# hyf015/egocentric-gaze-prediction

Hardware: AMD Instinct MI355X
Metric: SP+AT train frames/sec/node (224x224, bs32/GPU) (higher is better)
Workload: dtype f32 (every convolution -- forward, data gradient, weight gradient -- as f16 split-half MFMA, abs-max scaled operands, THREE products per MAC: 22 significant bits on both operands of every product; fp32 accumulate; everything else exact f32)

## Files before the change

### egocentric-gaze-prediction_amd/_lib.py

```python
from __future__ import annotations

import ctypes
import os
from ctypes import c_char_p, c_double, c_float, c_int, c_long, c_size_t, c_void_p

_HERE = os.path.dirname(os.path.abspath(__file__))
LIB_PATH = os.environ.get("EGAZE_HIP_LIB") or os.path.join(_HERE, "csrc", "libegaze_hip.so")

P = c_void_p
S = c_void_p

SIGNATURES = {
    "egz_version": (c_char_p, []),
    "egz_last_error": (c_char_p, []),
    "egz_mfma_probe": (c_int, [P, P, c_int, c_int, S]),
    "egz_u8_center_of_mass": (c_int, [P, c_int, c_int, c_int, P, P, P, S]),
    "egz_bilinear_up": (c_int, [P, P, c_int, c_int, c_int, c_int, c_int, c_long, S]),
    "egz_pack_w3x3_elems": (c_size_t, [c_int, c_int, c_int]),
    "egz_pack_w3x3_ups_fwd": (c_int, [P, P, c_int, c_int, S]),
    "egz_pack_w3x3_ups_dgrad": (c_int, [P, P, c_int, c_int, S]),
    "egz_conv3x3_ups_dgrad": (c_int, [P, P, P, c_int, c_int, c_int, c_int, c_int, c_int, S]),
    "egz_pack_w3x3_fwd": (c_int, [P, P, c_int, c_int, S]),
    "egz_pack_w3x3_dgrad": (c_int, [P, P, c_int, c_int, S]),
    "egz_conv3x3_stat_rows": (c_int, [c_int, c_int, c_int, c_int, c_int]),
# ... 91 lines not shown
    "egz_gaze_gt_maps": (c_int, [P, c_int, c_int, c_int, P, c_int, P, P, P, c_int, P, P, P, c_int, c_int, c_int, c_int,
                                 P, P, P, S]),
    "egz_resize_linear_u8": (c_int, [P, c_int, c_int, c_int, c_int, c_int, c_int, c_int, P, P, P, P, P, S]),
    "egz_heatmap_overlay": (c_int, [P, c_int, c_int, c_int, P, P, c_int, c_int, c_int, P, P, P, P, P, P, S]),
    "egz_cell_argmax_u8": (c_int, [P, c_int, c_int, c_int, c_int, P, S]),
    "egz_jpeg_decode_ws_bytes": (c_size_t, [c_int, c_int, c_int, c_int]),
    "egz_jpeg_decode": (c_int, [P, c_long, P, P, P, c_int, c_int, c_int, P, c_long, P, P, c_size_t, c_int, c_int, S]),
    "egz_jpeg_encode_ws_bytes": (c_size_t, [c_int, c_int, c_int, c_int]),
    "egz_jpeg_encode": (c_int, [P, c_int, c_int, c_int, c_int, c_int, c_int, P, c_size_t, P, c_int, S]),
    "egz_jpeg_encode_write": (c_int, [P, c_size_t, c_int, c_int, c_int, c_int, P, c_long, P, P, P, P, S]),
    "egz_tvl1_default_k": (c_int, []),
    "egz_bgr_to_gray_u8": (c_int, [P, c_int, c_int, c_int, c_int, P, S]),
    "egz_flow_gauss": (c_int, [P, c_int, c_int, c_int, c_int, P, c_int, P, P, S]),
    "egz_flow_resample": (c_int, [P, c_int, c_int, c_int, P, c_int, c_int, c_float, S]),
    "egz_flow_grad": (c_int, [P, c_int, c_int, c_int, P, P, S]),
    "egz_tvl1_warp": (c_int, [P, P, P, P, P, c_int, c_int, c_int, S]),
    "egz_tvl1_iterate": (c_int, [P, P, P, c_int, c_int, c_int, c_int, c_int, c_double, c_double, c_double, S]),
    "egz_flow_to_u8": (c_int, [P, c_long, c_double, P, S]),
    "egz_tvl1_flow_ws_bytes": (c_size_t, [c_int, c_int, c_int, c_int, c_double]),
    "egz_tvl1_flow": (c_int, [P, c_int, c_int, c_int, P, c_int, P, c_int, c_double, c_double, c_double, c_int, c_double,
                              c_int, c_int, c_int, P, c_size_t, P, P, S]),
    "egz_adam_step": (c_int, [P, P, P, P, c_long, c_double, c_double, c_double, c_double, c_int, c_double, P, S]),
    "egz_adam_step_dev": (c_int, [P, P, P, P, c_long, c_double, c_double, c_double, c_double, P, c_double, P, S]),
}


class EgazeHipError(RuntimeError):
    """Raised when a C-ABI entry point returns a non-zero code (mirrors the reference's convention of
    plain Python exceptions: utils.generalException / RuntimeError, SURVEY.md 8b)."""


def _load():
    if not os.path.exists(LIB_PATH):
        raise ImportError(
            f"{LIB_PATH} is missing: the HIP extension is mandatory (no CPU fallback). "
            "Build it with `python __graft_entry__.py` or `csrc/build.sh`.")
    import torch
    lib = ctypes.CDLL(LIB_PATH)
    for name, (res, args) in SIGNATURES.items():
        try:
            fn = getattr(lib, name)
        except AttributeError as e:
            raise ImportError(f"{LIB_PATH} does not export {name}; rebuild the extension") from e
        fn.restype = res
        fn.argtypes = args
    return lib
# ... 14 lines not shown
```

### egocentric-gaze-prediction_amd/csrc/adam.hip

```cpp
#include "egz_common.h"

namespace {
__global__ __launch_bounds__(256) void adam_kernel(float* __restrict__ p, const float* __restrict__ g, float* __restrict__ m,
                                                   float* __restrict__ v, long n, float omb1, float beta2, float omb2, float eps,
                                                   float step_size, float bc2_sqrt, float grad_scale,
                                                   unsigned int* __restrict__ nonfinite) {
#pragma clang fp contract(off)
    const long n4 = n >> 2;
    bool bad = false;
    for (long i = blockIdx.x * (long)blockDim.x + threadIdx.x; i < n4; i += (long)gridDim.x * blockDim.x) {
        f32x4 pv = reinterpret_cast<f32x4*>(p)[i];
        const f32x4 gv = reinterpret_cast<const f32x4*>(g)[i];
        f32x4 mv = reinterpret_cast<f32x4*>(m)[i];
        f32x4 vv = reinterpret_cast<f32x4*>(v)[i];
#pragma unroll
        for (int e = 0; e < 4; ++e) {
            const float ge = gv[e] * grad_scale;
            if (!(fabsf(ge) <= 3.402823466e38f)) { bad = true; continue; }
            mv[e] = mv[e] + omb1 * (ge - mv[e]);
            vv[e] = vv[e] * beta2 + omb2 * ge * ge;
            const float denom = sqrtf(vv[e]) / bc2_sqrt + eps;
            pv[e] = pv[e] - step_size * (mv[e] / denom);
        }
        reinterpret_cast<f32x4*>(p)[i] = pv;
        reinterpret_cast<f32x4*>(m)[i] = mv;
        reinterpret_cast<f32x4*>(v)[i] = vv;
    }
    const long t = n4 * 4 + blockIdx.x * (long)blockDim.x + threadIdx.x;
    if (t < n) {
        const float ge = g[t] * grad_scale;
        if (!(fabsf(ge) <= 3.402823466e38f)) bad = true;
        else {
            const float mm = m[t] + omb1 * (ge - m[t]);
            const float vq = v[t] * beta2 + omb2 * ge * ge;
            m[t] = mm;
            v[t] = vq;
            p[t] = p[t] - step_size * (mm / (sqrtf(vq) / bc2_sqrt + eps));
        }
    }
    if (bad && nonfinite) atomicOr(nonfinite, 1u);
}
__global__ __launch_bounds__(256) void adam_dev_kernel(float* __restrict__ p, const float* __restrict__ g, float* __restrict__ m,
                                                       float* __restrict__ v, long n, double lr, double beta1, double beta2,
                                                       float eps, int* __restrict__ step, float grad_scale,
                                                       unsigned int* __restrict__ nonfinite) {
#pragma clang fp contract(off)
    bool bad = false;
    const double t = (double)(*static_cast<volatile int*>(step) + 1);
    const float omb1 = (float)(1.0 - beta1), b2 = (float)beta2, omb2 = (float)(1.0 - beta2);
    const float step_size = (float)(lr / (1.0 - pow(beta1, t)));
    const float bc2_sqrt = (float)sqrt(1.0 - pow(beta2, t));
    const long n4 = n >> 2;
    for (long i = blockIdx.x * (long)blockDim.x + threadIdx.x; i < n4; i += (long)gridDim.x * blockDim.x) {
        f32x4 pv = reinterpret_cast<f32x4*>(p)[i];
        const f32x4 gv = reinterpret_cast<const f32x4*>(g)[i];
        f32x4 mv = reinterpret_cast<f32x4*>(m)[i];
        f32x4 vv = reinterpret_cast<f32x4*>(v)[i];
#pragma unroll
        for (int e = 0; e < 4; ++e) {
            const float ge = gv[e] * grad_scale;
            if (!(fabsf(ge) <= 3.402823466e38f)) { bad = true; continue; }
            mv[e] = mv[e] + omb1 * (ge - mv[e]);
            vv[e] = vv[e] * b2 + omb2 * ge * ge;
            const float denom = sqrtf(vv[e]) / bc2_sqrt + eps;
            pv[e] = pv[e] - step_size * (mv[e] / denom);
        }
        reinterpret_cast<f32x4*>(p)[i] = pv;
        reinterpret_cast<f32x4*>(m)[i] = mv;
        reinterpret_cast<f32x4*>(v)[i] = vv;
    }
    const long tl = n4 * 4 + blockIdx.x * (long)blockDim.x + threadIdx.x;
    if (tl < n) {
        const float ge = g[tl] * grad_scale;
        if (!(fabsf(ge) <= 3.402823466e38f)) bad = true;
        else {
            const float mm = m[tl] + omb1 * (ge - m[tl]);
            const float vq = v[tl] * b2 + omb2 * ge * ge;
            m[tl] = mm;
            v[tl] = vq;
            p[tl] = p[tl] - step_size * (mm / (sqrtf(vq) / bc2_sqrt + eps));
        }
    }
    if (bad && nonfinite) atomicOr(nonfinite, 1u);
}
__global__ void adam_bump_kernel(int* step) { *step += 1; }
}

EGZ_API int egz_adam_step_dev(float* p, const float* g, float* m, float* v, long n, double lr, double beta1, double beta2,
                              double eps, int* step, double grad_scale, unsigned int* nonfinite, hipStream_t st) {
    EGZ_CHECK_ARG(p && g && m && v && step && n > 0, "egz_adam_step_dev: bad arguments");
    EGZ_CHECK_ARG(((uintptr_t)p % 16 == 0) && ((uintptr_t)g % 16 == 0) && ((uintptr_t)m % 16 == 0) && ((uintptr_t)v % 16 == 0),
                  "egz_adam_step_dev: buffers must be 16-byte aligned");
    long g4 = (n / 4 + 255) / 256;
    if (g4 < 1) g4 = 1;
    const int grid = (int)(g4 > 8192 ? 8192 : g4);
    hipLaunchKernelGGL(adam_dev_kernel, dim3(grid), dim3(256), 0, st, p, g, m, v, n, lr, beta1, beta2, (float)eps, step,
                       (float)grad_scale, nonfinite);
    EGZ_CHECK_LAUNCH("egz_adam_step_dev");
    hipLaunchKernelGGL(adam_bump_kernel, dim3(1), dim3(1), 0, st, step);
    EGZ_CHECK_LAUNCH("egz_adam_step_dev(bump)");
    return 0;
}

EGZ_API int egz_adam_step(float* p, const float* g, float* m, float* v, long n, double lr, double beta1, double beta2,
                          double eps, int step, double grad_scale, unsigned int* nonfinite, hipStream_t st) {
    EGZ_CHECK_ARG(p && g && m && v && n > 0 && step >= 1, "egz_adam_step: bad arguments");
    EGZ_CHECK_ARG(((uintptr_t)p % 16 == 0) && ((uintptr_t)g % 16 == 0) && ((uintptr_t)m % 16 == 0) && ((uintptr_t)v % 16 == 0),
                  "egz_adam_step: buffers must be 16-byte aligned");
    const double bc1 = 1.0 - pow(beta1, (double)step);
    const double bc2 = 1.0 - pow(beta2, (double)step);
    const float step_size = (float)(lr / bc1);
    const float bc2_sqrt = (float)sqrt(bc2);
    long g4 = (n / 4 + 255) / 256;
    if (g4 < 1) g4 = 1;
    const int grid = (int)(g4 > 8192 ? 8192 : g4);
    hipLaunchKernelGGL(adam_kernel, dim3(grid), dim3(256), 0, st, p, g, m, v, n,
                       (float)(1.0 - beta1), (float)beta2, (float)(1.0 - beta2), (float)eps, step_size, bc2_sqrt, (float)grad_scale, nonfinite);
    EGZ_CHECK_LAUNCH("egz_adam_step");
    return 0;
}
```

### egocentric-gaze-prediction_amd/csrc/conv3x3_igemm_x3s.hip

```cpp
#include "egz_common.h"
#include "x3_split.h"
#include <type_traits>



namespace {
using namespace x3;

enum { EPI_BIAS = 0, EPI_BIAS_RELU = 1, EPI_BIAS_STATS = 2, EPI_MASK_SUMS = 3, EPI_PARTIAL = 4, EPI_BNSUMS = 5 };
constexpr int XLD = 32;
constexpr int XBK = 32;
constexpr int HPITCH = 20;

template <int WM> struct Geo {
    static constexpr int WMM = WM;
    static constexpr int NWN = 4 / WM;
    static constexpr int NTHR = 64 * WMM * NWN;
    static constexpr int MR = (WM == 4) ? 2 : 4;
    static constexpr int RPW = 32 * MR;
    static constexpr int BM = RPW * WMM, BN = 32 * NWN;
    static constexpr int HSLOTS = (WM == 1) ? 256 : 384, HZERO = HSLOTS - 1;
    static constexpr int NABUF = (WM == 1) ? 2 : 1;
    static constexpr int PROWS = BM / 16;
    static constexpr int SPP = NTHR / 8;
// ... 550 lines not shown
            const long srow = (long)tile_m * G::WMM + wm;
            if (hl == 0 && nok && srow * 128 < M) {
                stat[(srow * 2 + 0) * K + col] = s1;
                stat[(srow * 2 + 1) * K + col] = s2;
            }
        } else {
            if (hl == 0) {
                sred[(wave * 2 + 0) * 32 + l31] = s1;
                sred[(wave * 2 + 1) * 32 + l31] = s2;
            }
            lds_barrier();
            const long srow = (long)tile_m * (BM / 128) + (wm >> 1);
            if ((wm & 1) == 0 && hl == 0 && nok && srow * 128 < M) {
                stat[(srow * 2 + 0) * K + col] = s1 + sred[((wave + NWN) * 2 + 0) * 32 + l31];
                stat[(srow * 2 + 1) * K + col] = s2 + sred[((wave + NWN) * 2 + 1) * 32 + l31];
            }
        }
    }
#ifdef EGZ_TILE_LOOP
    }
#endif
}

__device__ __forceinline__ float weff9s(const float* __restrict__ w9, int py, int a, int px, int b) {
    const int rlo = (py == 0) ? (a == 0 ? 0 : 1) : (a == 0 ? 0 : 2), rhi = (py == 0) ? (a == 0 ? 0 : 2) : (a == 0 ? 1 : 2);
    const int slo = (px == 0) ? (b == 0 ? 0 : 1) : (b == 0 ? 0 : 2), shi = (px == 0) ? (b == 0 ? 0 : 2) : (b == 0 ? 1 : 2);
    float s = 0.f;
    for (int r = rlo; r <= rhi; ++r)
        for (int q = slo; q <= shi; ++q) s += w9[r * 3 + q];
    return s;
}

__device__ __forceinline__ float frag_value9(const float* w9, int kind, int si) {
    if (kind == 4) return w9[si];
    if (kind == 5) return w9[8 - si];
    if (kind == 7) return weff9s(w9, (si >> 2) >> 1, (si & 3) >> 1, (si >> 2) & 1, si & 1);
    const int img = si >> 2, tap = si & 3;
    const int oy = 2 * (tap >> 1) - (img >> 1), ox = 2 * (tap & 1) - (img & 1);
    return weff9s(w9, (oy == -1 || oy == 1) ? 1 : 0, (oy <= 0) ? 1 : 0, (ox == -1 || ox == 1) ? 1 : 0, (ox <= 0) ? 1 : 0);
}

template <typename T, int KIND>
__device__ __forceinline__ void frag_pack_pair(const float* __restrict__ w, unsigned short* __restrict__ wq, int C, int K,
                                               int Np, int Rp, float scale, long j) {
    constexpr int NS = (KIND >= 6) ? 16 : 9;
    const int nt32 = Np >> 5, ncb = Rp / XBK;
    const int e = (int)(j & 7), lane = (int)((j >> 3) & 63), ks = (int)((j >> 9) & 1);
    const long r2 = j >> 10;
    const int ntile = (int)(r2 % nt32), cblk = (int)(r2 / nt32);
    const int col = ntile * 32 + (lane & 31), k = cblk * XBK + ks * 16 + (lane >> 5) * 8 + e;
    float w9[9];
    const bool fwd = (KIND == 4 || KIND == 7);
    const bool ok = fwd ? (col < K && k < C) : (col < C && k < K);
    const float* src = w + (fwd ? ((long)col * C + k) : ((long)k * C + col)) * 9;
#pragma unroll
    for (int t = 0; t < 9; ++t) w9[t] = ok ? src[t] : 0.f;
#pragma unroll
    for (int si = 0; si < NS; ++si) {
        const long s = (KIND == 7) ? (long)(si >> 2) * (ncb * 4) + cblk * 4 + (si & 3) : (long)cblk * NS + si;
        const long r = s * nt32 + ntile;
        unsigned short h, l;
        Half<T>::split(frag_value9(w9, KIND, si) * scale, h, l);
        const long base = ((r * 2 + ks) * 2) * 512 + lane * 8 + e;
        wq[base] = h;
        wq[base + 512] = l;
    }
}
template <typename T>
__device__ __forceinline__ void frag_pack_pair_k(const float* __restrict__ w, unsigned short* __restrict__ wq, int C, int K,
                                                 int kind, int Np, int Rp, float scale, long j) {
    if (kind == 4) frag_pack_pair<T, 4>(w, wq, C, K, Np, Rp, scale, j);
    else if (kind == 5) frag_pack_pair<T, 5>(w, wq, C, K, Np, Rp, scale, j);
    else if (kind == 6) frag_pack_pair<T, 6>(w, wq, C, K, Np, Rp, scale, j);
    else frag_pack_pair<T, 7>(w, wq, C, K, Np, Rp, scale, j);
}

template <typename T>
__global__ __launch_bounds__(256) void pack_split_frag_kernel(const float* __restrict__ w, unsigned short* __restrict__ wq,
                                                             int C, int K, int kind, int Np, int Rp, float scale) {
    const long n = (long)Np * Rp;
    for (long j = blockIdx.x * (long)blockDim.x + threadIdx.x; j < n; j += (long)gridDim.x * blockDim.x)
        frag_pack_pair_k<T>(w, wq, C, K, kind, Np, Rp, scale, j);
}


constexpr int PT_LD = 289;
template <typename T>
__device__ __forceinline__ void pack_frag_tile(const float* __restrict__ w, unsigned short* __restrict__ wq, int C, int K,
                                               int kind, float scale, int tile, float* __restrict__ sw) {
    const int Cp = (C + 31) & ~31, Kp = (K + 31) & ~31;
    const int ncbc = Cp >> 5;
    const int kb = tile / ncbc, cb = tile - kb * ncbc;
    const int tid = threadIdx.x;
    if (C % 32 == 0 && (reinterpret_cast<unsigned long long>(w) & 15) == 0) {
        for (int idx = tid; idx < 32 * 72; idx += 256) {
            const int i = idx / 72, q = idx - i * 72;
            const int k = kb * 32 + i;
            f32x4 v = f32x4{0.f, 0.f, 0.f, 0.f};
            if (k < K) v = *reinterpret_cast<const f32x4*>(w + ((long)k * C + cb * 32) * 9 + q * 4);
            float* d = sw + i * PT_LD + q * 4;
            d[0] = v[0]; d[1] = v[1]; d[2] = v[2]; d[3] = v[3];
        }
    } else {
        for (int idx = tid; idx < 32 * 288; idx += 256) {
            const int i = idx / 288, q = idx - i * 288;
            const int k = kb * 32 + i, c = cb * 32 + q / 9;
            sw[i * PT_LD + q] = (k < K && c < C) ? w[(long)k * C * 9 + cb * 288 + q] : 0.f;
        }
    }
    __syncthreads();
    const bool fwd = (kind == 4 || kind == 7);
    const int NS = (kind >= 6) ? 16 : 9;
    const int nt32 = (fwd ? Kp : Cp) >> 5, ncb = (fwd ? Cp : Kp) >> 5;
    const int ntile = fwd ? kb : cb, cblk = fwd ? cb : kb;
    for (int it = tid; it < NS * 128; it += 256) {
        const int lane = it & 63, ks = (it >> 6) & 1, si = it >> 7;
        const int col = lane & 31, kk0 = ks * 16 + (lane >> 5) * 8;
        const float* p = fwd ? sw + col * PT_LD + kk0 * 9 : sw + kk0 * PT_LD + col * 9;
        const int estep = fwd ? 9 : PT_LD;
        unsigned short h[8], l[8];
#pragma unroll
        for (int e = 0; e < 8; ++e) {
            const float* pe = p + e * estep;
            float v;
            if (kind == 4) v = pe[si];
            else if (kind == 5) v = pe[8 - si];
            else {
                float w9[9];
#pragma unroll
                for (int t = 0; t < 9; ++t) w9[t] = pe[t];
                v = frag_value9(w9, kind, si);
            }
            Half<T>::split(v * scale, h[e], l[e]);
        }
        const long s = (kind == 7) ? (long)(si >> 2) * (ncb * 4) + cblk * 4 + (si & 3) : (long)cblk * NS + si;
        const long r = s * nt32 + ntile;
        const long base = ((r * 2 + ks) * 2) * 512 + lane * 8;
        u32x4 hv, lv;
#pragma unroll
        for (int e = 0; e < 4; ++e) {
            hv[e] = (unsigned)h[2 * e] | ((unsigned)h[2 * e + 1] << 16);
            lv[e] = (unsigned)l[2 * e] | ((unsigned)l[2 * e + 1] << 16);
        }
        *reinterpret_cast<u32x4*>(wq + base) = hv;
        *reinterpret_cast<u32x4*>(wq + base + 512) = lv;
    }
}

__global__ __launch_bounds__(256) void pack_frag_batch_kernel(const long long* __restrict__ table, int n) {
    __shared__ float sw[32 * PT_LD];
    const int b = (int)blockIdx.x;
    int lo = 0, hi = n - 1;
    while (lo < hi) {
        const int mid = (lo + hi + 1) >> 1;
        if (table[mid * 8 + 6] <= b) lo = mid; else hi = mid - 1;
    }
    const long long* d = table + lo * 8;
    const float* w = reinterpret_cast<const float*>(d[0]);
    unsigned short* wq = reinterpret_cast<unsigned short*>(d[1]);
    const int C = (int)d[2], K = (int)d[3], kind = (int)d[4], tile = b - (int)d[6];
    if (d[5] == 1) pack_frag_tile<_Float16>(w, wq, C, K, kind, F16_WSCALE, tile, sw);
    else pack_frag_tile<__bf16>(w, wq, C, K, kind, 1.f, tile, sw);
}


template <typename T, int EPI, bool BNIN>
__global__ __launch_bounds__(256, 1) void conv3x3_x3p_narrow_kernel(
    const float* __restrict__ x, const unsigned short* __restrict__ wq, const float* __restrict__ bias,
    float* __restrict__ y, double* __restrict__ stat, int B, int H, int W, int C, int K, float out_scale, int total,
    const unsigned int* __restrict__ a_absmax, const float* __restrict__ bn_y, const float* __restrict__ bn_coef,
// ... 665 lines not shown
```

### egocentric-gaze-prediction_amd/hipops.py

```python
from __future__ import annotations

import weakref
from typing import Optional, Tuple

import torch

from ._lib import LIB as _RAW_LIB, check

EPI_BIAS, EPI_BIAS_RELU, EPI_BIAS_STATS = 0, 1, 2
import os as _os


class _Profiler:

    def __init__(self):
        self.enabled = False
        self.events = {}
        self.flops = {}

    def start(self):
        self.events, self.flops, self.enabled = {}, {}, True

    def stop(self):
        self.enabled = False
# ... 219 lines not shown
    if ent is None and capturing:
        for key, w, buf in todo:
            check(LIB.egz_pack_w3x3_split_frag(w.data_ptr(), buf.data_ptr(), w.shape[1], w.shape[0], _PACK_FN[key[1]][2], key[2],
                                               _stream()), "egz_pack_w3x3_split_frag")
    else:
        if ent is None:
            rows, nb = [], 0
            for key, w, buf in todo:
                K, C = w.shape[0], w.shape[1]
                rows.append([w.data_ptr(), buf.data_ptr(), C, K, _PACK_FN[key[1]][2], key[2], nb, 0])
                nb += LIB.egz_pack_w3x3_frag_blocks(C, K)
            if len(_BATCH_TABLES) > 64:
                for k_ in [k_ for k_ in _BATCH_TABLES if k_ not in _BATCH_PINNED]:
                    del _BATCH_TABLES[k_]
            ent = (torch.tensor(rows, dtype=torch.int64).to(todo[0][1].device), nb)
            _BATCH_TABLES[sig] = ent
        if capturing:
            _BATCH_PINNED.add(sig)
        check(LIB.egz_pack_w3x3_frag_batch(ent[0].data_ptr(), len(todo), ent[1], _stream()), "egz_pack_w3x3_frag_batch")
    for key, w, buf in todo:
        _PACKED[key] = (_tag(w), buf, weakref.ref(w))
        _USED.discard(key)
    return len(todo)


def repack_stale(params) -> int:
    ids = {getattr(p, "_egz_uid", None) for p in params}
    n = 0
    for key in [k for k in _PACKED if k[0] in ids]:
        hit = _PACKED.get(key)
        w = hit[2]() if hit is not None else None
        if w is not None and hit[0] != _tag(w):
            packed_weight(w, key[1], key[2])
            n += 1
    return n


class GradSink:
    __slots__ = ("buf", "owner", "gen_written", "hooks")

    def __init__(self, buf, owner):
        self.buf, self.owner, self.gen_written, self.hooks = buf, owner, -1, []


def grad_sink(param, wanted: bool = True) -> Optional[torch.Tensor]:
    if not wanted:
# ... 2015 lines not shown
```

### egocentric-gaze-prediction_amd/optim.py

```python
from __future__ import annotations

from typing import Iterable, List

import os

import torch

from . import hipops as H
from . import streams




class FusedAdam:
    def __init__(self, params, lr: float = 1e-3, betas=(0.9, 0.999), eps: float = 1e-8):
        params = list(params)
        if params and isinstance(params[0], dict):
            if len(params) != 1:
                raise NotImplementedError("the reference uses a single parameter group")
            group = params[0]
            lr = group.get("lr", lr)
            params = list(group["params"])
        self.params: List[torch.nn.Parameter] = [p for p in params if p.requires_grad]
        if not self.params:
# ... 48 lines not shown

    def zero_grad(self, set_to_none: bool = False, all_overwritten: bool = False):
        from . import functions as _F
        _F._JOIN_QUEUED[0] = False
        if all_overwritten:
            pass
        else:
            H.fill_zero(self.flat_g)
        self.zero_gen += 1
        for p, o in zip(self.params, self.offsets):
            if p.grad is None or p.grad.data_ptr() != self.flat_g.data_ptr() + 4 * o:
                p.grad = self.flat_g[o:o + p.numel()].view(p.shape)

    @torch.no_grad()
    def step(self):
        from . import functions as _F
        _F._JOIN_QUEUED[0] = False
        for hook in self.pre_step_hooks:
            hook()
        capturing = torch.cuda.is_current_stream_capturing()
        if not capturing:
            streams.join_all_into_current()
        self.step_count += 1
        if self.capturable:
            H.adam_step_dev(self.flat_p, self.flat_g, self.flat_m, self.flat_v, self.lr, self.betas[0], self.betas[1],
                            self.eps, self.step_dev, self.grad_scale, nonfinite=self.nonfinite)
        else:
            if capturing:
                raise RuntimeError("FusedAdam.step() inside a hipGraph capture needs set_capturable(True)")
            H.adam_step(self.flat_p, self.flat_g, self.flat_m, self.flat_v, self.lr, self.betas[0], self.betas[1],
                        self.eps, self.step_count, self.grad_scale, nonfinite=self.nonfinite)
        H.touch_params(self.params)
        H.refresh_packings(self.params)

    @property
    def param_groups(self):
        return [dict(self.defaults, lr=self.lr, maximize=False, foreach=None, capturable=False, differentiable=False,
                     fused=None, decoupled_weight_decay=False, params=list(range(len(self.params))))]

    def state_dict(self):
        state = {}
        if self.step_count > 0:
            for i, (p, o) in enumerate(zip(self.params, self.offsets)):
                n = p.numel()
                state[i] = {"step": torch.tensor(float(self.step_count)),
                            "exp_avg": self.flat_m[o:o + n].view(p.shape).clone(),
                            "exp_avg_sq": self.flat_v[o:o + n].view(p.shape).clone()}
        return {"state": state, "param_groups": self.param_groups}

    def load_state_dict(self, sd):
        groups = sd.get("param_groups", [])
        if groups and "params" in groups[0] and len(groups[0]["params"]) != len(self.params):
            raise ValueError("loaded state dict contains a parameter group that doesn't match the size of "
                             "optimizer's group")
# ... 19 lines not shown
```

### include/egaze_hip.h

```cpp
#ifndef EGAZE_HIP_H
#define EGAZE_HIP_H

#include <stddef.h>

#ifdef __cplusplus
extern "C" {
#endif

typedef struct ihipStream_t* hipStream_t;

const char* egz_version(void);
const char* egz_last_error(void);

size_t egz_pack_w3x3_elems(int C, int K, int kind );
int egz_pack_w3x3_fwd(const float* w, float* wp, int C, int K, hipStream_t stream);
int egz_pack_w3x3_dgrad(const float* w, float* wp, int C, int K, hipStream_t stream);
int egz_pack_w3x3_ups_fwd(const float* w, float* wp, int C, int K, hipStream_t stream);
int egz_pack_w3x3_ups_dgrad(const float* w, float* wp, int C, int K, hipStream_t stream);
int egz_conv3x3_stat_rows(int B, int H, int W, int K, int flags);
int egz_conv3x3_fwd(const float* x, const float* wp, const float* bias, float* y, double* stat_partial, int B, int H,
                    int W, int C, int K, int flags, hipStream_t stream);
int egz_conv3x3_ups_dgrad(const float* dy, const float* wp, float* dx, int B, int H, int W, int C, int K, int flags,
                          hipStream_t stream);
int egz_pack_w3x3_split(const float* w, void* wp, int C, int K, int kind, int dtype, hipStream_t stream);
// ... 125 lines not shown
                         const float* const* b_hh, const float* h0, const float* c0, float* hs, float* cs, float* acts, float* hn,
                         float* cn, unsigned int* sync, int L, int T, int B, int H, hipStream_t stream);
int egz_lstm_wave_bwd(const float* dh_top, const float* dhn, const float* dcn, const float* acts, const float* cs,
                      const float* c0, const float* const* w_hh_t, const float* const* w_ih_t, float* dgates, float* dh0,
                      float* dc0, float* dhin, int L, int T, int B, int H, hipStream_t stream);
int egz_lstm_persist_bwd(const float* dh_top, const float* dhn, const float* dcn, const float* acts, const float* cs,
                         const float* c0, const float* const* w_hh, const float* const* w_ih, float* dgates, float* dh0,
                         float* dc0, float* const* db, unsigned int* sync, int L, int T, int B, int H, hipStream_t stream);
size_t egz_lstm_b1_ws_bytes(int L, int C, int H, int N);
int egz_lstm_b1_fwd(const void* const* params, int L, const float* inp, const float* h0, const float* c0, float* xt,
                    float* acts, float* hn, float* cn, float* out, int C, int H, int N, hipStream_t stream);
int egz_lstm_b1_bwd(const void* const* params, void* const* grads, int L, const float* dout, const float* dhn,
                    const float* dcn, const float* xt, const float* acts, const float* h0, const float* c0,
                    const float* hn, const float* cn, const float* out, int C, int H, int N, void* workspace,
                    size_t ws_bytes, hipStream_t stream);
int egz_tanh_fwd(const float* x, float* y, long n, hipStream_t stream);
int egz_tanh_bwd(const float* y, const float* dy, float* dx, long n, hipStream_t stream);
int egz_add(const float* a, const float* b, float* out, long n, hipStream_t stream);

int egz_adam_step(float* p, const float* g, float* m, float* v, long n, double lr, double beta1, double beta2,
                  double eps, int step, double grad_scale, unsigned int* nonfinite, hipStream_t stream);
int egz_adam_step_dev(float* p, const float* g, float* m, float* v, long n, double lr, double beta1, double beta2,
                      double eps, int* step, double grad_scale, unsigned int* nonfinite, hipStream_t stream);

int egz_aae_auc(const float* out, const float* gt, int B, int H, int W, const double* gw, int R, double dist,
                double* res, hipStream_t stream);

int egz_gaze_gt_maps(const int* pos, int N, int H, int W, const double* gw, int R, const int* xofs, const int* xsi,
                     const float* xalpha, int nx, const int* yofs, const int* ysi, const float* yalpha, int ny, int mode,
                     int oh, int ow, unsigned char* out_u8, double* out_f64, double* out_full, hipStream_t stream);

int egz_resize_linear_u8(const unsigned char* src, int N, int C, int sh, int sw, int dh, int dw, int interleaved,
                         const int* xofs, const short* xalpha, const int* yofs, const short* yalpha, unsigned char* dst,
                         hipStream_t stream);
int egz_heatmap_overlay(const unsigned char* maps, int M, int h, int w, const int* frame_index, const unsigned char* frames,
                        int F, int H, int W, const unsigned char* lut, const int* xofs, const short* xalpha, const int* yofs,
                        const short* yalpha, unsigned char* out, hipStream_t stream);
int egz_cell_argmax_u8(const unsigned char* gt, int N, int H, int W, int cell, int* out, hipStream_t stream);

size_t egz_jpeg_decode_ws_bytes(int N, int H, int W, int n3);
int egz_jpeg_decode(const unsigned char* data, long data_len, const long* offsets, const int* channels, const long* planes,
                    int N, int H, int W, unsigned char* out, long out_planes, int* status, void* ws, size_t ws_bytes,
                    int n3, int stages, hipStream_t stream);

size_t egz_jpeg_encode_ws_bytes(int N, int H, int W, int C);
int egz_jpeg_encode(const unsigned char* images, int N, int H, int W, int C, int quality, int subsampling, void* ws,
// ... 43 lines not shown
```

Measured before the change: 1090.

## Fuse Adam update with split-half conv weight repacking into one kernel

Adds a fused optimizer kernel that applies the Adam update to the flat parameter buffer and, for 3x3 conv weights with stale MFMA packings, writes the updated tile to shared memory and emits the packed f16/bf16 split fragments straight from it. A per-signature block table maps blocks either to plain ranges or to weight tiles. This removes the separate repack pass, which re-read every updated weight from global memory and cost extra launches after each step. In exchange there is a binary-search dispatch per block, extra table bookkeeping in Python, and a fallback to the old path whenever the layout assumptions fail.

```diff
diff --git a/egocentric-gaze-prediction_amd/_lib.py b/egocentric-gaze-prediction_amd/_lib.py
--- a/egocentric-gaze-prediction_amd/_lib.py
+++ b/egocentric-gaze-prediction_amd/_lib.py
@@ -137,6 +137,10 @@
                               c_int, c_int, c_int, P, c_size_t, P, P, S]),
     "egz_adam_step": (c_int, [P, P, P, P, c_long, c_double, c_double, c_double, c_double, c_int, c_double, P, S]),
     "egz_adam_step_dev": (c_int, [P, P, P, P, c_long, c_double, c_double, c_double, c_double, P, c_double, P, S]),
+    "egz_adam_pack_range_blocks": (c_int, [c_long]),
+    "egz_adam_pack_max_packings": (c_int, []),
+    "egz_adam_pack_step": (c_int, [P, P, P, P, c_double, c_double, c_double, c_double, c_int, c_double, P, P, c_int, c_int, S]),
+    "egz_adam_pack_step_dev": (c_int, [P, P, P, P, c_double, c_double, c_double, c_double, P, c_double, P, P, c_int, c_int, S]),
 }
 
 
diff --git a/egocentric-gaze-prediction_amd/csrc/adam.hip b/egocentric-gaze-prediction_amd/csrc/adam.hip
--- a/egocentric-gaze-prediction_amd/csrc/adam.hip
+++ b/egocentric-gaze-prediction_amd/csrc/adam.hip
@@ -1,86 +1,18 @@
 #include "egz_common.h"
+#include "adam_update.h"
 
 namespace {
 __global__ __launch_bounds__(256) void adam_kernel(float* __restrict__ p, const float* __restrict__ g, float* __restrict__ m,
-                                                   float* __restrict__ v, long n, float omb1, float beta2, float omb2, float eps,
-                                                   float step_size, float bc2_sqrt, float grad_scale,
-                                                   unsigned int* __restrict__ nonfinite) {
-#pragma clang fp contract(off)
-    const long n4 = n >> 2;
-    bool bad = false;
-    for (long i = blockIdx.x * (long)blockDim.x + threadIdx.x; i < n4; i += (long)gridDim.x * blockDim.x) {
-        f32x4 pv = reinterpret_cast<f32x4*>(p)[i];
-        const f32x4 gv = reinterpret_cast<const f32x4*>(g)[i];
-        f32x4 mv = reinterpret_cast<f32x4*>(m)[i];
-        f32x4 vv = reinterpret_cast<f32x4*>(v)[i];
-#pragma unroll
-        for (int e = 0; e < 4; ++e) {
-            const float ge = gv[e] * grad_scale;
-            if (!(fabsf(ge) <= 3.402823466e38f)) { bad = true; continue; }
-            mv[e] = mv[e] + omb1 * (ge - mv[e]);
-            vv[e] = vv[e] * beta2 + omb2 * ge * ge;
-            const float denom = sqrtf(vv[e]) / bc2_sqrt + eps;
-            pv[e] = pv[e] - step_size * (mv[e] / denom);
-        }
-        reinterpret_cast<f32x4*>(p)[i] = pv;
-        reinterpret_cast<f32x4*>(m)[i] = mv;
-        reinterpret_cast<f32x4*>(v)[i] = vv;
-    }
-    const long t = n4 * 4 + blockIdx.x * (long)blockDim.x + threadIdx.x;
-    if (t < n) {
-        const float ge = g[t] * grad_scale;
-        if (!(fabsf(ge) <= 3.402823466e38f)) bad = true;
-        else {
-            const float mm = m[t] + omb1 * (ge - m[t]);
-            const float vq = v[t] * beta2 + omb2 * ge * ge;
-            m[t] = mm;
-            v[t] = vq;
-            p[t] = p[t] - step_size * (mm / (sqrtf(vq) / bc2_sqrt + eps));
-        }
-    }
+                                                   float* __restrict__ v, long n, AdamCoef c, unsigned int* __restrict__ nonfinite) {
+    const bool bad = adam_range(p, g, m, v, n, blockIdx.x * (long)blockDim.x + threadIdx.x, (long)gridDim.x * blockDim.x, c);
     if (bad && nonfinite) atomicOr(nonfinite, 1u);
 }
 __global__ __launch_bounds__(256) void adam_dev_kernel(float* __restrict__ p, const float* __restrict__ g, float* __restrict__ m,
                                                        float* __restrict__ v, long n, double lr, double beta1, double beta2,
                                                        float eps, int* __restrict__ step, float grad_scale,
                                                        unsigned int* __restrict__ nonfinite) {
-#pragma clang fp contract(off)
-    bool bad = false;
-    const double t = (double)(*static_cast<volatile int*>(step) + 1);
-    const float omb1 = (float)(1.0 - beta1), b2 = (float)beta2, omb2 = (float)(1.0 - beta2);
-    const float step_size = (float)(lr / (1.0 - pow(beta1, t)));
-    const float bc2_sqrt = (float)sqrt(1.0 - pow(beta2, t));
-    const long n4 = n >> 2;
-    for (long i = blockIdx.x * (long)blockDim.x + threadIdx.x; i < n4; i += (long)gridDim.x * blockDim.x) {
-        f32x4 pv = reinterpret_cast<f32x4*>(p)[i];
-        const f32x4 gv = reinterpret_cast<const f32x4*>(g)[i];
-        f32x4 mv = reinterpret_cast<f32x4*>(m)[i];
-        f32x4 vv = reinterpret_cast<f32x4*>(v)[i];
-#pragma unroll
-        for (int e = 0; e < 4; ++e) {
-            const float ge = gv[e] * grad_scale;
-            if (!(fabsf(ge) <= 3.402823466e38f)) { bad = true; continue; }
-            mv[e] = mv[e] + omb1 * (ge - mv[e]);
-            vv[e] = vv[e] * b2 + omb2 * ge * ge;
-            const float denom = sqrtf(vv[e]) / bc2_sqrt + eps;
-            pv[e] = pv[e] - step_size * (mv[e] / denom);
-        }
-        reinterpret_cast<f32x4*>(p)[i] = pv;
-        reinterpret_cast<f32x4*>(m)[i] = mv;
-        reinterpret_cast<f32x4*>(v)[i] = vv;
-    }
-    const long tl = n4 * 4 + blockIdx.x * (long)blockDim.x + threadIdx.x;
-    if (tl < n) {
-        const float ge = g[tl] * grad_scale;
-        if (!(fabsf(ge) <= 3.402823466e38f)) bad = true;
-        else {
-            const float mm = m[tl] + omb1 * (ge - m[tl]);
-            const float vq = v[tl] * b2 + omb2 * ge * ge;
-            m[tl] = mm;
-            v[tl] = vq;
-            p[tl] = p[tl] - step_size * (mm / (sqrtf(vq) / bc2_sqrt + eps));
-        }
-    }
+    const AdamCoef c = adam_coef_dev(lr, beta1, beta2, eps, step, grad_scale);
+    const bool bad = adam_range(p, g, m, v, n, blockIdx.x * (long)blockDim.x + threadIdx.x, (long)gridDim.x * blockDim.x, c);
     if (bad && nonfinite) atomicOr(nonfinite, 1u);
 }
 __global__ void adam_bump_kernel(int* step) { *step += 1; }
@@ -107,15 +39,11 @@
     EGZ_CHECK_ARG(p && g && m && v && n > 0 && step >= 1, "egz_adam_step: bad arguments");
     EGZ_CHECK_ARG(((uintptr_t)p % 16 == 0) && ((uintptr_t)g % 16 == 0) && ((uintptr_t)m % 16 == 0) && ((uintptr_t)v % 16 == 0),
                   "egz_adam_step: buffers must be 16-byte aligned");
-    const double bc1 = 1.0 - pow(beta1, (double)step);
-    const double bc2 = 1.0 - pow(beta2, (double)step);
-    const float step_size = (float)(lr / bc1);
-    const float bc2_sqrt = (float)sqrt(bc2);
     long g4 = (n / 4 + 255) / 256;
     if (g4 < 1) g4 = 1;
     const int grid = (int)(g4 > 8192 ? 8192 : g4);
     hipLaunchKernelGGL(adam_kernel, dim3(grid), dim3(256), 0, st, p, g, m, v, n,
-                       (float)(1.0 - beta1), (float)beta2, (float)(1.0 - beta2), (float)eps, step_size, bc2_sqrt, (float)grad_scale, nonfinite);
+                       adam_coef_host(lr, beta1, beta2, eps, step, grad_scale), nonfinite);
     EGZ_CHECK_LAUNCH("egz_adam_step");
     return 0;
 }
diff --git a/egocentric-gaze-prediction_amd/csrc/adam_pack.hip b/egocentric-gaze-prediction_amd/csrc/adam_pack.hip
--- /dev/null
+++ b/egocentric-gaze-prediction_amd/csrc/adam_pack.hip
@@ -0,0 +1,134 @@
+#include "egz_common.h"
+#include "adam_update.h"
+#include "x3_pack.h"
+
+namespace {
+using namespace x3;
+
+constexpr int AP_MAX_PACK = 4;
+constexpr int AP_COLS = 6 + 2 * AP_MAX_PACK;
+constexpr int AP_CHUNK = 4096;
+
+__device__ __forceinline__ void adam_pack_block(float* __restrict__ p, const float* __restrict__ g, float* __restrict__ m,
+                                                float* __restrict__ v, const long long* __restrict__ table, int n,
+                                                const AdamCoef& c, unsigned int* __restrict__ nonfinite, float* __restrict__ sw) {
+    const int b = (int)blockIdx.x, tid = threadIdx.x;
+    int lo = 0, hi = n - 1;
+    while (lo < hi) {
+        const int mid = (lo + hi + 1) >> 1;
+        if (table[mid * AP_COLS + 4] <= b) lo = mid; else hi = mid - 1;
+    }
+    const long long* d = table + lo * AP_COLS;
+    const long off = d[1];
+    const int rel = b - (int)d[4];
+    bool bad = false;
+    if (d[0] == 0) {
+        const long start = (long)rel * AP_CHUNK, left = d[2] - start;
+        if (left > 0) {
+            const long o = off + start;
+            bad = adam_range(p + o, g + o, m + o, v + o, left < AP_CHUNK ? left : AP_CHUNK, tid, 256, c);
+        }
+    } else {
+        const int C = (int)d[2], K = (int)d[3];
+        const int ncbc = (C + 31) >> 5;
+        const int kb = rel / ncbc, cb = rel - kb * ncbc;
+        if (kb * 32 >= K) return;
+        if (C % 32 == 0 && (reinterpret_cast<unsigned long long>(p + off) & 15) == 0) {
+#pragma unroll 3
+            for (int idx = tid; idx < 32 * 72; idx += 256) {
+                const int i = idx / 72, q = idx - i * 72;
+                const int k = kb * 32 + i;
+                f32x4 pv = f32x4{0.f, 0.f, 0.f, 0.f};
+                if (k < K) {
+                    const long o = off + ((long)k * C + cb * 32) * 9 + q * 4;
+                    pv = *reinterpret_cast<const f32x4*>(p + o);
+                    const f32x4 gv = *reinterpret_cast<const f32x4*>(g + o);
+                    f32x4 mv = *reinterpret_cast<const f32x4*>(m + o);
+                    f32x4 vv = *reinterpret_cast<const f32x4*>(v + o);
+                    bad |= adam_update4(pv, gv, mv, vv, c);
+                    *reinterpret_cast<f32x4*>(p + o) = pv;
+                    *reinterpret_cast<f32x4*>(m + o) = mv;
+                    *reinterpret_cast<f32x4*>(v + o) = vv;
+                }
+                float* s = sw + i * PT_LD + q * 4;
+                s[0] = pv[0]; s[1] = pv[1]; s[2] = pv[2]; s[3] = pv[3];
+            }
+        } else {
+            for (int idx = tid; idx < 32 * 288; idx += 256) {
+                const int i = idx / 288, q = idx - i * 288;
+                const int k = kb * 32 + i, ch = cb * 32 + q / 9;
+                float pe = 0.f;
+                if (k < K && ch < C) {
+                    const long o = off + (long)k * C * 9 + cb * 288 + q;
+                    pe = p[o];
+                    float me = m[o], ve = v[o];
+                    if (adam_update(pe, g[o], me, ve, c)) { p[o] = pe; m[o] = me; v[o] = ve; }
+                    else bad = true;
+                }
+                sw[i * PT_LD + q] = pe;
+            }
+        }
+        __syncthreads();
+        const int np = (int)d[5];
+        for (int j = 0; j < np; ++j) {
+            unsigned short* wq = reinterpret_cast<unsigned short*>(d[6 + j]);
+            const int kd = (int)d[6 + AP_MAX_PACK + j], kind = kd & 0xff;
+            if ((kd >> 8) == 1) pack_frag_tile_emit<_Float16>(wq, C, K, kind, F16_WSCALE, rel, sw);
+            else pack_frag_tile_emit<__bf16>(wq, C, K, kind, 1.f, rel, sw);
+        }
+    }
+    if (bad && nonfinite) atomicOr(nonfinite, 1u);
+}
+
+__global__ __launch_bounds__(256) void adam_pack_kernel(float* __restrict__ p, const float* __restrict__ g, float* __restrict__ m,
+                                                        float* __restrict__ v, const long long* __restrict__ table, int n,
+                                                        AdamCoef c, unsigned int* __restrict__ nonfinite) {
+    __shared__ float sw[32 * PT_LD];
+    adam_pack_block(p, g, m, v, table, n, c, nonfinite, sw);
+}
+__global__ __launch_bounds__(256) void adam_pack_dev_kernel(float* __restrict__ p, const float* __restrict__ g, float* __restrict__ m,
+                                                            float* __restrict__ v, const long long* __restrict__ table, int n,
+                                                            double lr, double beta1, double beta2, float eps,
+                                                            const int* __restrict__ step, float grad_scale,
+                                                            unsigned int* __restrict__ nonfinite) {
+    __shared__ float sw[32 * PT_LD];
+    const AdamCoef c = adam_coef_dev(lr, beta1, beta2, eps, step, grad_scale);
+    adam_pack_block(p, g, m, v, table, n, c, nonfinite, sw);
+}
+__global__ void adam_pack_bump_kernel(int* step) { *step += 1; }
+
+int check_args(const char* who, const float* p, const float* g, const float* m, const float* v, const long long* table, int rows,
+               int total_blocks) {
+    EGZ_CHECK_ARG(p && g && m && v && table && rows > 0 && total_blocks >= rows, "%s: bad arguments", who);
+    EGZ_CHECK_ARG(((uintptr_t)p % 16 == 0) && ((uintptr_t)g % 16 == 0) && ((uintptr_t)m % 16 == 0) && ((uintptr_t)v % 16 == 0) &&
+                  ((uintptr_t)table % 8 == 0), "%s: buffers must be 16-byte aligned", who);
+    return 0;
+}
+}
+
+EGZ_API int egz_adam_pack_range_blocks(long n) { return n > 0 ? (int)((n + AP_CHUNK - 1) / AP_CHUNK) : 0; }
+EGZ_API int egz_adam_pack_max_packings(void) { return AP_MAX_PACK; }
+
+EGZ_API int egz_adam_pack_step(float* p, const float* g, float* m, float* v, double lr, double beta1, double beta2, double eps,
+                               int step, double grad_scale, unsigned int* nonfinite, const long long* table, int rows,
+                               int total_blocks, hipStream_t st) {
+    if (int rc = check_args("egz_adam_pack_step", p, g, m, v, table, rows, total_blocks)) return rc;
+    EGZ_CHECK_ARG(step >= 1, "egz_adam_pack_step: bad arguments");
+    hipLaunchKernelGGL(adam_pack_kernel, dim3(total_blocks), dim3(256), 0, st, p, g, m, v, table, rows,
+                       adam_coef_host(lr, beta1, beta2, eps, step, grad_scale), nonfinite);
+    EGZ_CHECK_LAUNCH("egz_adam_pack_step");
+    return 0;
+}
+
+EGZ_API int egz_adam_pack_step_dev(float* p, const float* g, float* m, float* v, double lr, double beta1, double beta2, double eps,
+                                   int* step, double grad_scale, unsigned int* nonfinite, const long long* table, int rows,
+                                   int total_blocks, hipStream_t st) {
+    if (int rc = check_args("egz_adam_pack_step_dev", p, g, m, v, table, rows, total_blocks)) return rc;
+    EGZ_CHECK_ARG(step != nullptr, "egz_adam_pack_step_dev: bad arguments");
+    hipLaunchKernelGGL(adam_pack_dev_kernel, dim3(total_blocks), dim3(256), 0, st, p, g, m, v, table, rows, lr, beta1, beta2,
+                       (float)eps, step, (float)grad_scale, nonfinite);
+    EGZ_CHECK_LAUNCH("egz_adam_pack_step_dev");
+    hipLaunchKernelGGL(adam_pack_bump_kernel, dim3(1), dim3(1), 0, st, step);
+    EGZ_CHECK_LAUNCH("egz_adam_pack_step_dev(bump)");
+    return 0;
+}
diff --git a/egocentric-gaze-prediction_amd/csrc/adam_update.h b/egocentric-gaze-prediction_amd/csrc/adam_update.h
--- /dev/null
+++ b/egocentric-gaze-prediction_amd/csrc/adam_update.h
@@ -0,0 +1,62 @@
+#pragma once
+#include "egz_common.h"
+
+struct AdamCoef {
+    float omb1, beta2, omb2, eps, step_size, bc2_sqrt, grad_scale;
+};
+
+static inline AdamCoef adam_coef_host(double lr, double beta1, double beta2, double eps, int step, double grad_scale) {
+    const double bc1 = 1.0 - pow(beta1, (double)step);
+    const double bc2 = 1.0 - pow(beta2, (double)step);
+    return AdamCoef{(float)(1.0 - beta1), (float)beta2, (float)(1.0 - beta2), (float)eps, (float)(lr / bc1), (float)sqrt(bc2),
+                    (float)grad_scale};
+}
+__device__ __forceinline__ AdamCoef adam_coef_dev(double lr, double beta1, double beta2, float eps, const int* step,
+                                                  float grad_scale) {
+    const double t = (double)(*static_cast<const volatile int*>(step) + 1);
+    return AdamCoef{(float)(1.0 - beta1), (float)beta2, (float)(1.0 - beta2), eps, (float)(lr / (1.0 - pow(beta1, t))),
+                    (float)sqrt(1.0 - pow(beta2, t)), grad_scale};
+}
+
+__device__ __forceinline__ bool adam_update(float& p, const float g, float& m, float& v, const AdamCoef& c) {
+#pragma clang fp contract(off)
+    const float ge = g * c.grad_scale;
+    if (!(fabsf(ge) <= 3.402823466e38f)) return false;
+    m = m + c.omb1 * (ge - m);
+    v = v * c.beta2 + c.omb2 * ge * ge;
+    const float denom = sqrtf(v) / c.bc2_sqrt + c.eps;
+    p = p - c.step_size * (m / denom);
+    return true;
+}
+__device__ __forceinline__ bool adam_update4(f32x4& p, const f32x4 g, f32x4& m, f32x4& v, const AdamCoef& c) {
+    bool bad = false;
+#pragma unroll
+    for (int e = 0; e < 4; ++e) {
+        float pe = p[e], me = m[e], ve = v[e];
+        if (adam_update(pe, g[e], me, ve, c)) { p[e] = pe; m[e] = me; v[e] = ve; }
+        else bad = true;
+    }
+    return bad;
+}
+__device__ __forceinline__ bool adam_range(float* __restrict__ p, const float* __restrict__ g, float* __restrict__ m,
+                                           float* __restrict__ v, long n, long first, long stride, const AdamCoef& c) {
+    bool bad = false;
+    const long n4 = n >> 2;
+    for (long i = first; i < n4; i += stride) {
+        f32x4 pv = reinterpret_cast<f32x4*>(p)[i];
+        const f32x4 gv = reinterpret_cast<const f32x4*>(g)[i];
+        f32x4 mv = reinterpret_cast<f32x4*>(m)[i];
+        f32x4 vv = reinterpret_cast<f32x4*>(v)[i];
+        bad |= adam_update4(pv, gv, mv, vv, c);
+        reinterpret_cast<f32x4*>(p)[i] = pv;
+        reinterpret_cast<f32x4*>(m)[i] = mv;
+        reinterpret_cast<f32x4*>(v)[i] = vv;
+    }
+    const long t = n4 * 4 + first;
+    if (t < n) {
+        float pe = p[t], me = m[t], ve = v[t];
+        if (adam_update(pe, g[t], me, ve, c)) { m[t] = me; v[t] = ve; p[t] = pe; }
+        else bad = true;
+    }
+    return bad;
+}
diff --git a/egocentric-gaze-prediction_amd/csrc/conv3x3_igemm_x3s.hip b/egocentric-gaze-prediction_amd/csrc/conv3x3_igemm_x3s.hip
--- a/egocentric-gaze-prediction_amd/csrc/conv3x3_igemm_x3s.hip
+++ b/egocentric-gaze-prediction_amd/csrc/conv3x3_igemm_x3s.hip
@@ -1,5 +1,6 @@
 #include "egz_common.h"
 #include "x3_split.h"
+#include "x3_pack.h"
 #include <type_traits>
 
 
@@ -596,24 +597,6 @@
 #endif
 }
 
-__device__ __forceinline__ float weff9s(const float* __restrict__ w9, int py, int a, int px, int b) {
-    const int rlo = (py == 0) ? (a == 0 ? 0 : 1) : (a == 0 ? 0 : 2), rhi = (py == 0) ? (a == 0 ? 0 : 2) : (a == 0 ? 1 : 2);
-    const int slo = (px == 0) ? (b == 0 ? 0 : 1) : (b == 0 ? 0 : 2), shi = (px == 0) ? (b == 0 ? 0 : 2) : (b == 0 ? 1 : 2);
-    float s = 0.f;
-    for (int r = rlo; r <= rhi; ++r)
-        for (int q = slo; q <= shi; ++q) s += w9[r * 3 + q];
-    return s;
-}
-
-__device__ __forceinline__ float frag_value9(const float* w9, int kind, int si) {
-    if (kind == 4) return w9[si];
-    if (kind == 5) return w9[8 - si];
-    if (kind == 7) return weff9s(w9, (si >> 2) >> 1, (si & 3) >> 1, (si >> 2) & 1, si & 1);
-    const int img = si >> 2, tap = si & 3;
-    const int oy = 2 * (tap >> 1) - (img >> 1), ox = 2 * (tap & 1) - (img & 1);
-    return weff9s(w9, (oy == -1 || oy == 1) ? 1 : 0, (oy <= 0) ? 1 : 0, (ox == -1 || ox == 1) ? 1 : 0, (ox <= 0) ? 1 : 0);
-}
-
 template <typename T, int KIND>
 __device__ __forceinline__ void frag_pack_pair(const float* __restrict__ w, unsigned short* __restrict__ wq, int C, int K,
                                                int Np, int Rp, float scale, long j) {
@@ -657,69 +640,6 @@
         frag_pack_pair_k<T>(w, wq, C, K, kind, Np, Rp, scale, j);
 }
 
-
-constexpr int PT_LD = 289;
-template <typename T>
-__device__ __forceinline__ void pack_frag_tile(const float* __restrict__ w, unsigned short* __restrict__ wq, int C, int K,
-                                               int kind, float scale, int tile, float* __restrict__ sw) {
-    const int Cp = (C + 31) & ~31, Kp = (K + 31) & ~31;
-    const int ncbc = Cp >> 5;
-    const int kb = tile / ncbc, cb = tile - kb * ncbc;
-    const int tid = threadIdx.x;
-    if (C % 32 == 0 && (reinterpret_cast<unsigned long long>(w) & 15) == 0) {
-        for (int idx = tid; idx < 32 * 72; idx += 256) {
-            const int i = idx / 72, q = idx - i * 72;
-            const int k = kb * 32 + i;
-            f32x4 v = f32x4{0.f, 0.f, 0.f, 0.f};
-            if (k < K) v = *reinterpret_cast<const f32x4*>(w + ((long)k * C + cb * 32) * 9 + q * 4);
-            float* d = sw + i * PT_LD + q * 4;
-            d[0] = v[0]; d[1] = v[1]; d[2] = v[2]; d[3] = v[3];
-        }
-    } else {
-        for (int idx = tid; idx < 32 * 288; idx += 256) {
-            const int i = idx / 288, q = idx - i * 288;
-            const int k = kb * 32 + i, c = cb * 32 + q / 9;
-            sw[i * PT_LD + q] = (k < K && c < C) ? w[(long)k * C * 9 + cb * 288 + q] : 0.f;
-        }
-    }
-    __syncthreads();
-    const bool fwd = (kind == 4 || kind == 7);
-    const int NS = (kind >= 6) ? 16 : 9;
-    const int nt32 = (fwd ? Kp : Cp) >> 5, ncb = (fwd ? Cp : Kp) >> 5;
-    const int ntile = fwd ? kb : cb, cblk = fwd ? cb : kb;
-    for (int it = tid; it < NS * 128; it += 256) {
-        const int lane = it & 63, ks = (it >> 6) & 1, si = it >> 7;
-        const int col = lane & 31, kk0 = ks * 16 + (lane >> 5) * 8;
-        const float* p = fwd ? sw + col * PT_LD + kk0 * 9 : sw + kk0 * PT_LD + col * 9;
-        const int estep = fwd ? 9 : PT_LD;
-        unsigned short h[8], l[8];
-#pragma unroll
-        for (int e = 0; e < 8; ++e) {
-            const float* pe = p + e * estep;
-            float v;
-            if (kind == 4) v = pe[si];
-            else if (kind == 5) v = pe[8 - si];
-            else {
-                float w9[9];
-#pragma unroll
-                for (int t = 0; t < 9; ++t) w9[t] = pe[t];
-                v = frag_value9(w9, kind, si);
-            }
-            Half<T>::split(v * scale, h[e], l[e]);
-        }
-        const long s = (kind == 7) ? (long)(si >> 2) * (ncb * 4) + cblk * 4 + (si & 3) : (long)cblk * NS + si;
-        const long r = s * nt32 + ntile;
-        const long base = ((r * 2 + ks) * 2) * 512 + lane * 8;
-        u32x4 hv, lv;
-#pragma unroll
-        for (int e = 0; e < 4; ++e) {
-            hv[e] = (unsigned)h[2 * e] | ((unsigned)h[2 * e + 1] << 16);
-            lv[e] = (unsigned)l[2 * e] | ((unsigned)l[2 * e + 1] << 16);
-        }
-        *reinterpret_cast<u32x4*>(wq + base) = hv;
-        *reinterpret_cast<u32x4*>(wq + base + 512) = lv;
-    }
-}
 
 __global__ __launch_bounds__(256) void pack_frag_batch_kernel(const long long* __restrict__ table, int n) {
     __shared__ float sw[32 * PT_LD];
diff --git a/egocentric-gaze-prediction_amd/csrc/x3_pack.h b/egocentric-gaze-prediction_amd/csrc/x3_pack.h
--- /dev/null
+++ b/egocentric-gaze-prediction_amd/csrc/x3_pack.h
@@ -0,0 +1,99 @@
+#pragma once
+#include "x3_split.h"
+
+namespace x3 {
+
+__device__ __forceinline__ float weff9s(const float* __restrict__ w9, int py, int a, int px, int b) {
+    const int rlo = (py == 0) ? (a == 0 ? 0 : 1) : (a == 0 ? 0 : 2), rhi = (py == 0) ? (a == 0 ? 0 : 2) : (a == 0 ? 1 : 2);
+    const int slo = (px == 0) ? (b == 0 ? 0 : 1) : (b == 0 ? 0 : 2), shi = (px == 0) ? (b == 0 ? 0 : 2) : (b == 0 ? 1 : 2);
+    float s = 0.f;
+    for (int r = rlo; r <= rhi; ++r)
+        for (int q = slo; q <= shi; ++q) s += w9[r * 3 + q];
+    return s;
+}
+
+__device__ __forceinline__ float frag_value9(const float* w9, int kind, int si) {
+    if (kind == 4) return w9[si];
+    if (kind == 5) return w9[8 - si];
+    if (kind == 7) return weff9s(w9, (si >> 2) >> 1, (si & 3) >> 1, (si >> 2) & 1, si & 1);
+    const int img = si >> 2, tap = si & 3;
+    const int oy = 2 * (tap >> 1) - (img >> 1), ox = 2 * (tap & 1) - (img & 1);
+    return weff9s(w9, (oy == -1 || oy == 1) ? 1 : 0, (oy <= 0) ? 1 : 0, (ox == -1 || ox == 1) ? 1 : 0, (ox <= 0) ? 1 : 0);
+}
+
+constexpr int PT_LD = 289;
+__device__ __forceinline__ void pack_frag_tile_load(const float* __restrict__ w, int C, int K, int tile, float* __restrict__ sw) {
+    const int Cp = (C + 31) & ~31;
+    const int ncbc = Cp >> 5;
+    const int kb = tile / ncbc, cb = tile - kb * ncbc;
+    const int tid = threadIdx.x;
+    if (C % 32 == 0 && (reinterpret_cast<unsigned long long>(w) & 15) == 0) {
+        for (int idx = tid; idx < 32 * 72; idx += 256) {
+            const int i = idx / 72, q = idx - i * 72;
+            const int k = kb * 32 + i;
+            f32x4 v = f32x4{0.f, 0.f, 0.f, 0.f};
+            if (k < K) v = *reinterpret_cast<const f32x4*>(w + ((long)k * C + cb * 32) * 9 + q * 4);
+            float* d = sw + i * PT_LD + q * 4;
+            d[0] = v[0]; d[1] = v[1]; d[2] = v[2]; d[3] = v[3];
+        }
+    } else {
+        for (int idx = tid; idx < 32 * 288; idx += 256) {
+            const int i = idx / 288, q = idx - i * 288;
+            const int k = kb * 32 + i, c = cb * 32 + q / 9;
+            sw[i * PT_LD + q] = (k < K && c < C) ? w[(long)k * C * 9 + cb * 288 + q] : 0.f;
+        }
+    }
+}
+template <typename T>
+__device__ __forceinline__ void pack_frag_tile_emit(unsigned short* __restrict__ wq, int C, int K, int kind, float scale, int tile,
+                                                    const float* __restrict__ sw) {
+    const int Cp = (C + 31) & ~31, Kp = (K + 31) & ~31;
+    const int ncbc = Cp >> 5;
+    const int kb = tile / ncbc, cb = tile - kb * ncbc;
+    const int tid = threadIdx.x;
+    const bool fwd = (kind == 4 || kind == 7);
+    const int NS = (kind >= 6) ? 16 : 9;
+    const int nt32 = (fwd ? Kp : Cp) >> 5, ncb = (fwd ? Cp : Kp) >> 5;
+    const int ntile = fwd ? kb : cb, cblk = fwd ? cb : kb;
+    for (int it = tid; it < NS * 128; it += 256) {
+        const int lane = it & 63, ks = (it >> 6) & 1, si = it >> 7;
+        const int col = lane & 31, kk0 = ks * 16 + (lane >> 5) * 8;
+        const float* p = fwd ? sw + col * PT_LD + kk0 * 9 : sw + kk0 * PT_LD + col * 9;
+        const int estep = fwd ? 9 : PT_LD;
+        unsigned short h[8], l[8];
+#pragma unroll
+        for (int e = 0; e < 8; ++e) {
+            const float* pe = p + e * estep;
+            float v;
+            if (kind == 4) v = pe[si];
+            else if (kind == 5) v = pe[8 - si];
+            else {
+                float w9[9];
+#pragma unroll
+                for (int t = 0; t < 9; ++t) w9[t] = pe[t];
+                v = frag_value9(w9, kind, si);
+            }
+            Half<T>::split(v * scale, h[e], l[e]);
+        }
+        const long s = (kind == 7) ? (long)(si >> 2) * (ncb * 4) + cblk * 4 + (si & 3) : (long)cblk * NS + si;
+        const long r = s * nt32 + ntile;
+        const long base = ((r * 2 + ks) * 2) * 512 + lane * 8;
+        u32x4 hv, lv;
+#pragma unroll
+        for (int e = 0; e < 4; ++e) {
+            hv[e] = (unsigned)h[2 * e] | ((unsigned)h[2 * e + 1] << 16);
+            lv[e] = (unsigned)l[2 * e] | ((unsigned)l[2 * e + 1] << 16);
+        }
+        *reinterpret_cast<u32x4*>(wq + base) = hv;
+        *reinterpret_cast<u32x4*>(wq + base + 512) = lv;
+    }
+}
+template <typename T>
+__device__ __forceinline__ void pack_frag_tile(const float* __restrict__ w, unsigned short* __restrict__ wq, int C, int K,
+                                               int kind, float scale, int tile, float* __restrict__ sw) {
+    pack_frag_tile_load(w, C, K, tile, sw);
+    __syncthreads();
+    pack_frag_tile_emit<T>(wq, C, K, kind, scale, tile, sw);
+}
+
+}
diff --git a/egocentric-gaze-prediction_amd/hipops.py b/egocentric-gaze-prediction_amd/hipops.py
--- a/egocentric-gaze-prediction_amd/hipops.py
+++ b/egocentric-gaze-prediction_amd/hipops.py
@@ -265,6 +265,81 @@
         _PACKED[key] = (_tag(w), buf, weakref.ref(w))
         _USED.discard(key)
     return len(todo)
+
+
+FUSED_STEP = True
+_STEP_TABLES = {}
+_STEP_PINNED = set()
+
+
+def adam_pack_step(params, offsets, p, g, m, v, lr, beta1, beta2, eps, step, grad_scale=1.0, nonfinite=None, step_dev=None) -> bool:
+    if not (FUSED_STEP and BATCH_REPACK) or not _USED:
+        return False
+    where = {getattr(q, "_egz_uid", None): i for i, q in enumerate(params)}
+    by_weight = {}
+    for key in sorted(k for k in _USED if k[0] in where and k[2] and _PACK_FN[k[1]][2] >= 4):
+        hit = _PACKED.get(key)
+        w = hit[2]() if hit is not None else None
+        if w is None:
+            _USED.discard(key)
+            continue
+        by_weight.setdefault(key[0], []).append((key, w, hit[1]))
+    if not by_weight:
+        return False
+    max_pack = _RAW_LIB.egz_adam_pack_max_packings()
+    for uid, packs in by_weight.items():
+        w, o = packs[0][1], offsets[where[uid]]
+        if (len(packs) > max_pack or w.numel() != w.shape[0] * w.shape[1] * 9 or w.numel() % 4 or o % 4 or not w.is_contiguous()
+                or w.data_ptr() != p.data_ptr() + 4 * o):
+            return False
+    todo = [t for uid in sorted(by_weight, key=lambda u: offsets[where[u]]) for t in by_weight[uid]]
+    sig = (p.data_ptr(), p.numel()) + tuple((key, w.data_ptr(), buf.data_ptr()) for key, w, buf in todo)
+    ent = _STEP_TABLES.get(sig)
+    capturing = torch.cuda.is_current_stream_capturing()
+    if ent is None:
+        if capturing:
+            return False
+        cols = 6 + 2 * max_pack
+        rows, nb, at = [], 0, 0
+
+        def range_row(lo, hi):
+            nonlocal nb
+            if hi > lo:
+                rows.append([0, lo, hi - lo, 0, nb, 0] + [0] * (2 * max_pack))
+                nb += _RAW_LIB.egz_adam_pack_range_blocks(hi - lo)
+
+        for uid in sorted(by_weight, key=lambda u: offsets[where[u]]):
+            packs = by_weight[uid]
+            w, o = packs[0][1], offsets[where[uid]]
+            K, C = w.shape[0], w.shape[1]
+            range_row(at, o)
+            pad = [0] * (max_pack - len(packs))
+            rows.append([1, o, C, K, nb, len(packs)] + [buf.data_ptr() for _, _, buf in packs] + pad
+                        + [_PACK_FN[key[1]][2] | (key[2] << 8) for key, _, _ in packs] + pad)
+            nb += _RAW_LIB.egz_pack_w3x3_frag_blocks(C, K)
+            at = o + w.numel()
+        range_row(at, p.numel())
+        assert all(len(r) == cols for r in rows)
+        if len(_STEP_TABLES) > 64:
+            for k_ in [k_ for k_ in _STEP_TABLES if k_ not in _STEP_PINNED]:
+                del _STEP_TABLES[k_]
+        ent = (torch.tensor(rows, dtype=torch.int64).to(p.device), len(rows), nb)
+        _STEP_TABLES[sig] = ent
+    if capturing:
+        _STEP_PINNED.add(sig)
+    if step_dev is not None:
+        check(LIB.egz_adam_pack_step_dev(p.data_ptr(), g.data_ptr(), m.data_ptr(), v.data_ptr(), lr, beta1, beta2, eps,
+                                         step_dev.data_ptr(), grad_scale, _p(nonfinite), ent[0].data_ptr(), ent[1], ent[2],
+                                         _stream()), "egz_adam_pack_step_dev")
+    else:
+        check(LIB.egz_adam_pack_step(p.data_ptr(), g.data_ptr(), m.data_ptr(), v.data_ptr(), lr, beta1, beta2, eps, int(step),
+                                     grad_scale, _p(nonfinite), ent[0].data_ptr(), ent[1], ent[2], _stream()),
+              "egz_adam_pack_step")
+    touch_params(params)
+    for key, w, buf in todo:
+        _PACKED[key] = (_tag(w), buf, weakref.ref(w))
+        _USED.discard(key)
+    return True
 
 
 def repack_stale(params) -> int:
diff --git a/egocentric-gaze-prediction_amd/optim.py b/egocentric-gaze-prediction_amd/optim.py
--- a/egocentric-gaze-prediction_amd/optim.py
+++ b/egocentric-gaze-prediction_amd/optim.py
@@ -94,14 +94,18 @@
         if not capturing:
             streams.join_all_into_current()
         self.step_count += 1
+        if not self.capturable and capturing:
+            raise RuntimeError("FusedAdam.step() inside a hipGraph capture needs set_capturable(True)")
+        hyper = (self.lr, self.betas[0], self.betas[1], self.eps)
+        if H.adam_pack_step(self.params, self.offsets, self.flat_p, self.flat_g, self.flat_m, self.flat_v, *hyper, self.step_count,
+                            self.grad_scale, nonfinite=self.nonfinite, step_dev=self.step_dev if self.capturable else None):
+            return
         if self.capturable:
-            H.adam_step_dev(self.flat_p, self.flat_g, self.flat_m, self.flat_v, self.lr, self.betas[0], self.betas[1],
-                            self.eps, self.step_dev, self.grad_scale, nonfinite=self.nonfinite)
+            H.adam_step_dev(self.flat_p, self.flat_g, self.flat_m, self.flat_v, *hyper, self.step_dev, self.grad_scale,
+                            nonfinite=self.nonfinite)
         else:
-            if capturing:
-                raise RuntimeError("FusedAdam.step() inside a hipGraph capture needs set_capturable(True)")
-            H.adam_step(self.flat_p, self.flat_g, self.flat_m, self.flat_v, self.lr, self.betas[0], self.betas[1],
-                        self.eps, self.step_count, self.grad_scale, nonfinite=self.nonfinite)
+            H.adam_step(self.flat_p, self.flat_g, self.flat_m, self.flat_v, *hyper, self.step_count, self.grad_scale,
+                        nonfinite=self.nonfinite)
         H.touch_params(self.params)
         H.refresh_packings(self.params)
 
diff --git a/include/egaze_hip.h b/include/egaze_hip.h
--- a/include/egaze_hip.h
+++ b/include/egaze_hip.h
@@ -171,6 +171,14 @@
                   double eps, int step, double grad_scale, unsigned int* nonfinite, hipStream_t stream);
 int egz_adam_step_dev(float* p, const float* g, float* m, float* v, long n, double lr, double beta1, double beta2,
                       double eps, int* step, double grad_scale, unsigned int* nonfinite, hipStream_t stream);
+int egz_adam_pack_range_blocks(long n);
+int egz_adam_pack_max_packings(void);
+int egz_adam_pack_step(float* p, const float* g, float* m, float* v, double lr, double beta1, double beta2, double eps,
+                       int step, double grad_scale, unsigned int* nonfinite, const long long* table, int rows,
+                       int total_blocks, hipStream_t stream);
+int egz_adam_pack_step_dev(float* p, const float* g, float* m, float* v, double lr, double beta1, double beta2, double eps,
+                           int* step, double grad_scale, unsigned int* nonfinite, const long long* table, int rows,
+                           int total_blocks, hipStream_t stream);
 
 int egz_aae_auc(const float* out, const float* gt, int B, int H, int W, const double* gw, int R, double dist,
                 double* res, hipStream_t stream);
```

Result: no change. 1080 (median of 2 runs) (-0.9%).
